# gabegrand/VQA-Counterexamples

Hardware: AMD Instinct MI355X
Metric: VQA-CX triplets/sec (24 candidates each), NeuralCX training step (higher is better)
Workload: dtype f32; 1 GPU; configs[1]: NeuralCX MLP train step (fwd+listwise loss/recall+bwd+Adam), synthetic 2048-d feats, 24 candidates, batch 512 per GPU (weak scaling: global batch 512), H=256, L=1, dropout 0.25, fp32; global_batch=512, per_rank_batch=512, candidates=24, dim_h=256, n_layers=1, parallelism=dp1, feature_table_rows=82783

## Files before the change

### include/neuralcx.h

```cpp
#ifndef NEURALCX_H
#define NEURALCX_H

#include <stddef.h>
#include <stdint.h>

#ifdef __cplusplus
extern "C" {
#endif

#define NCX_OK            0
#define NCX_E_NULL       -1
#define NCX_E_DIMS       -2
#define NCX_E_WORKSPACE  -3
#define NCX_E_FLAGS      -4
#define NCX_E_UNSUPPORTED -5
#define NCX_E_COMM       -6

#define NCX_F_V_MULT   (1u << 0)
#define NCX_F_V_DIST   (1u << 1)
#define NCX_F_V_RANK   (1u << 2)
#define NCX_F_A_EMB    (1u << 3)
#define NCX_F_ALL      (NCX_F_V_MULT | NCX_F_V_DIST | NCX_F_V_RANK | NCX_F_A_EMB)
#define NCX_F_BF16     (1u << 4)
#define NCX_F_REUSE_GT (1u << 5)
// ... 102 lines not shown
    int32_t act_v, act_q;
} ncx_mutan_params;

size_t ncx_vqa_workspace_bytes(const ncx_dims* d, const ncx_mutan_params* m);

int ncx_vqa_forward(const ncx_dims* d, const float* feats, const int32_t* img_idx, const float* q_emb,
                    const ncx_mutan_params* m, void* workspace, size_t workspace_bytes,
                    float* z_orig, float* z_knns, float* a_knns, float* a_orig, void* stream);

size_t ncx_knn_workspace_bytes(int32_t n, int32_t block_rows);
int ncx_knn(const float* table, int32_t n, const float* queries, int32_t nq, int32_t dv, int32_t k,
            int32_t norms_ready, void* workspace, size_t workspace_bytes, int64_t* out_idx, float* out_dist,
            void* stream);

size_t ncx_cosine_gram_workspace_bytes(int32_t A, int32_t da);
int ncx_cosine_gram(const float* emb, int32_t A, int32_t da, void* ws, size_t ws_bytes, float* gram, void* stream);
int ncx_semantic_scores(const float* a_knns, const int32_t* aid, int32_t B, int32_t K, int32_t A, const float* gram,
                        float lam, float* scores, float* raw, int32_t* bad_id_flag, void* stream);

#define NCX_GEMM_GT 0
#define NCX_GEMM_SH 1
#define NCX_GEMM_MAIN 2
#define NCX_GEMM_FWD_L 3
#define NCX_GEMM_DW1C 4
#define NCX_GEMM_DW1S 5
#define NCX_GEMM_DE 6
#define NCX_GEMM_DW1AK 7
#define NCX_GEMM_DAGT 8
#define NCX_GEMM_DWL 9
#define NCX_GEMM_DXL 10
int ncx_profile_begin(uint32_t gemm_mask , int32_t max_launches);
int ncx_profile_end(float* ms, int32_t* ids, int32_t cap);
int ncx_profile_stamps(unsigned long long* stamps, int64_t words);
int ncx_plan_query(const ncx_dims* d, int32_t gemm_id, int32_t* out6);
int ncx_wgmap_check(int32_t tiles_m, int32_t tiles_n, int32_t S);

const char* ncx_version(void);

#ifdef __cplusplus
}
#endif
#endif
```

### vqa-counterexamples_amd/csrc/ncx_api.hip

```cpp
#include "ncx_internal.h"
#include "ncx_dwred.h"
#include "ncx_bf16.h"
#include <stdlib.h>
#include <stdio.h>
#include <atomic>

namespace ncx {

template <int CTRL> __device__ __forceinline__ float dpp_mov(float v) {
    return __builtin_bit_cast(float, __builtin_amdgcn_update_dpp(0, __builtin_bit_cast(int, v), CTRL, 0xF, 0xF, false));
}
__device__ __forceinline__ float lane_bcast(float v, int lane) {
    return __builtin_bit_cast(float, __builtin_amdgcn_readlane(__builtin_bit_cast(int, v), lane));
}
__device__ __forceinline__ float wave_sum(float v) {
    v += dpp_mov<0xB1>(v); v += dpp_mov<0x4E>(v); v += dpp_mov<0x141>(v); v += dpp_mov<0x140>(v);
    return (lane_bcast(v, 0) + lane_bcast(v, 16)) + (lane_bcast(v, 32) + lane_bcast(v, 48));
}
__device__ __forceinline__ float wave_max(float v) {
    v = fmaxf(v, dpp_mov<0xB1>(v)); v = fmaxf(v, dpp_mov<0x4E>(v)); v = fmaxf(v, dpp_mov<0x141>(v)); v = fmaxf(v, dpp_mov<0x140>(v));
    return fmaxf(fmaxf(lane_bcast(v, 0), lane_bcast(v, 16)), fmaxf(lane_bcast(v, 32), lane_bcast(v, 48)));
}

__device__ __forceinline__ u16 f32_to_bf16(float x) { return __builtin_bit_cast(u16, (__bf16)x); }
// ... 717 lines not shown
    if (const char* e = hook_env("NCX_SMALL_COLS")) narrow = atoll(e);
    if (S <= 1 || cols > narrow) return S;
    int mult = 2;
    if (const char* e = hook_env("NCX_SMALL_MULT")) mult = atoi(e) > 0 ? atoi(e) : 1;
    long long sp = (long long)S * mult;
    const long long smax = ksteps / 8 > 1 ? ksteps / 8 : 1;
    if (sp > smax) sp = smax;
    return (int)(sp < S ? S : sp);
}

static void list_uses(const ncx_dims& d, GemmUse* u) {
    const long long M = (long long)d.B * d.K, H = d.H;
    const bool aemb = d.flags & NCX_F_A_EMB;
    const long long cand_k = ks(d.dv) * ((d.flags & NCX_F_V_MULT) ? 2 : 1) + ks(d.K + 1) + ks(d.dz) + (aemb ? ks(d.A) : ks(d.da));
    const long long cand_cols = (long long)d.dv * ((d.flags & NCX_F_V_MULT) ? 2 : 1) + d.K + 1 + d.dz + (aemb ? d.A : d.da);
    const long long sh_k = ks(d.dv) + ks(d.dq) + ks(d.dz) + ks(d.da);
    const long long sh_cols = (long long)d.dv + d.dq + d.dz + d.da;
    u[U_GT]    = {FORM_NT, H, d.A, ks(d.da), false};
    u[U_SH]    = {FORM_NT, d.B, H, sh_k, false};
    u[U_MAIN]  = {FORM_NT, M, H, cand_k, true};
    u[U_FWD_L] = {FORM_NT, M, H, ks(H), true};
    u[U_DW1C]  = {FORM_TN, H, cand_cols, ks(M), false};
    u[U_DW1S]  = {FORM_TN, H, sh_cols, ks(d.B), false};
    u[U_DE]    = {FORM_TN, d.A, d.da, 2 * ks(H), false};
    u[U_DW1AK] = {FORM_NN, H, d.da, ks(d.A), false};
    u[U_DAGT]  = {FORM_NN, 1, 1, 1, false};
    u[U_DWL]   = {FORM_TN, H, H, ks(M), false};
    u[U_DXL]   = {FORM_NN, M, H, ks(H), false};
    const bool hooks = experiment_hooks_on();
    for (int i = 0; i < U_COUNT; ++i) {
        const bool km = dw_km_supported(d) && !(d.flags & NCX_F_BF16);
        const bool tn8 = dw_tn8_supported(d);
        const long long segs_c[5] = {km ? 0 : d.dv, (!km && (d.flags & NCX_F_V_MULT)) ? d.dv : 0, tn8 ? 0 : d.K + 1, tn8 ? 0 : d.dz, tn8 ? 0 : (aemb ? d.A : d.da)};
        const bool tn8s = tn8 || dw_tn8_shapes_ok(d);
        const long long segs_s[5] = {tn8s ? 0 : d.dv, tn8s ? 0 : d.dq, tn8s ? 0 : d.dz, tn8s ? 0 : d.da, 0};
        const bool grouped = i == U_DW1C || i == U_DW1S;
        auto grouped_tiles = [&](int bm, int bn) {
            const long long* sg = i == U_DW1C ? segs_c : segs_s;
            long long t = 0;
            for (int q = 0; q < 5; ++q) t += cdiv(H, bm) * cdiv(sg[q], bn);
            return t;
        };
        if (grouped && grouped_tiles(64, 64) == 0) {
            u[i].plan.cfg = CFG_128x64; u[i].plan.split = 1;
        } else if (grouped) {
            u[i].plan = plan_from_tiles(FORM_TN, grouped_tiles(128, 128), grouped_tiles(64, 64), u[i].ksteps, false);
            if (i == U_DW1C && H >= 128 && u[i].plan.split > 1) {
                u[i].plan.cfg = CFG_128x64;
                const long long slots = (long long)occupancy_tn(CFG_128x64) * num_cus();
                long long sp = cdiv(3 * slots, grouped_tiles(128, 64));
                const long long smax = u[i].ksteps / 24 > 1 ? u[i].ksteps / 24 : 1;
                if (sp > 8) sp = 8;
                u[i].plan.split = (int)(sp > smax ? smax : sp < 1 ? 1 : sp);
            }
        } else {
            u[i].plan = plan_gemm(u[i].form, u[i].M, u[i].N, u[i].ksteps, u[i].allow96);
        }
        if (i == U_MAIN || i == U_FWD_L || i == U_DXL) u[i].plan.split = 1;
        if (hooks) {
            char name[32];
            snprintf(name, sizeof name, "NCX_CFG_%d", i);
            const char* c = getenv(name);
            if (c) u[i].plan.cfg = atoi(c);
            snprintf(name, sizeof name, "NCX_SPLIT_%d", i);
            const char* e = getenv(name);
            if (e && i != U_MAIN && i != U_FWD_L && i != U_DXL) u[i].plan.split = atoi(e) > 1 ? atoi(e) : 1;
        }
        int bm, bn; cfg_tile(u[i].plan.cfg, bm, bn);
        long long tiles = cdiv(u[i].M, bm) * cdiv(u[i].N, bn);
        if (grouped) tiles = grouped_tiles(bm, bn);
        u[i].tiles = tiles;
        const int S = u[i].plan.split > 1 ? u[i].plan.split : 1;
        long long wgs = 0;
        if (grouped) {
            const long long* sg = i == U_DW1C ? segs_c : segs_s;
            for (int q = 0; q < 5; ++q)
                if (sg[q] > 0) wgs += WgMap{(int)cdiv(H, bm), (int)cdiv(sg[q], bn), i == U_DW1C ? dw1c_seg_split(sg[q], S, u[i].ksteps) : S}.count();
        } else {
            wgs = WgMap{(int)cdiv(u[i].M, bm), (int)cdiv(u[i].N, bn), S}.count();
        }
        u[i].wgs = wgs;
        u[i].slab_elems = S > 1 ? wgs * bm * bn : 0;
    }
    u[U_DW1S].plan.cfg = u[U_DW1C].plan.cfg;
    {
        int bm, bn; cfg_tile(u[U_DW1C].plan.cfg, bm, bn);
        const bool tn8 = dw_tn8_shapes_ok(d);
        const long long segs_s[4] = {tn8 ? 0 : d.dv, tn8 ? 0 : d.dq, tn8 ? 0 : d.dz, tn8 ? 0 : d.da};
        const int S = u[U_DW1S].plan.split > 1 ? u[U_DW1S].plan.split : 1;
        u[U_DW1S].tiles = 0; u[U_DW1S].wgs = 0;
        for (int q = 0; q < 4; ++q) {
            if (segs_s[q] == 0) continue;
            u[U_DW1S].tiles += cdiv(H, bm) * cdiv(segs_s[q], bn);
            u[U_DW1S].wgs += WgMap{(int)cdiv(H, bm), (int)cdiv(segs_s[q], bn), S}.count();
        }
        u[U_DW1C].slab_elems = (u[U_DW1C].wgs + u[U_DW1S].wgs) * bm * bn;
        u[U_DW1S].slab_elems = 0;
    }
}

WsLayout ws_layout(const ncx_dims& d) {
    WsLayout w{};
    const size_t M = (size_t)d.B * d.K, H = d.H;
    size_t off = 0;
    auto take = [&](size_t bytes) { size_t o = off; off = align_up(off + bytes, 256); return o; };
    w.idx_k = take(M * 4); w.idx_o = take(M * 4); w.idx_ob = take((size_t)d.B * 4);
    w.mx = take(M * 4); w.inv = take(M * 4);
    w.ldm = pad_to(d.K + 1, 4);
    w.ldgt = (d.flags & NCX_F_BF16) ? d.A : pad_to(d.A, 32);
    w.misc = take(M * w.ldm * 4);
    w.gt = take(H * w.ldgt * 4);
    w.sh = take((size_t)d.B * H * 4);
    for (int l = 0; l < 3; ++l) w.h[l] = l < d.L ? take(M * H * 4) : 0;
    w.dpre[0] = take(M * H * 4);
    w.dpre[1] = d.L >= 2 ? take(M * H * 4) : 0;
    w.dsh = take((size_t)d.B * H * 4);
    w.dgt = take(2 * H * d.A * 4);
    w.dagt = w.dgt + H * d.A * 4;
    w.dgtT = take((size_t)2 * d.A * pad_to(d.H, 4) * 4);
    w.w1aT = take((size_t)2 * d.da * pad_to(d.H, 32) * 4);
// ... 628 lines not shown
            prob(in->q_emb, d.dq, 0, d.dq, g->w1 + o.q_emb);
            prob(in->z_orig, d.dz, 0, d.dz, g->w1 + o.z_orig);
            if (aemb) prob(p->answer_embedding, d.da, 2, d.da, g->w1 + o.a_gt);
            else      prob(in->a_emb_gt, d.da, 0, d.da, g->w1 + o.a_gt);
            rc = dw_tn8(d, tp, np, 0, false, true, idx_ob, aemb ? in->answer_aids : nullptr, slab, w.slab_bytes, s); if (rc) return rc;
        } else
        if (want_rest && !tn8) {
            add_s(x_gather(in->feats, d.dv, idx_ob, d.B, d.dv), g->w1 + o.v_orig);
            add_s(x_plain(in->q_emb, d.dq, d.B, d.dq), g->w1 + o.q_emb);
            add_s(x_plain(in->z_orig, d.dz, d.B, d.dz), g->w1 + o.z_orig);
            add_s(aemb ? x_gather(p->answer_embedding, d.da, in->answer_aids, d.B, d.da) : x_plain(in->a_emb_gt, d.da, d.B, d.da),
                  g->w1 + o.a_gt);
        }
        a.nseg = n;
        FixupArgs fix_tn{};
        if (km_merge) a.defer_fix = &fix_tn;
        if (n > 0) { rc = run_gemm(U_DW1C, a, FORM_TN, u[U_DW1C].plan, slab, w.slab_bytes, nullptr, s); if (rc) return rc; }
        if (km_merge && !km_reduced) {
            rc = prof_open(U_DW1C, s); if (rc) return rc;
            rc = dw_km_finish(d, (const float*)(ws + w.km_slab), g->w1 + o.v_other, g->w1 + o.v_mult, din, &fix_tn, u[U_DW1C].plan.cfg, s);
            if (rc) return rc;
            rc = prof_close(U_DW1C, s); if (rc) return rc;
        }
        if (!(d.flags & NCX_F_V_MULT) && do2) {
            hipLaunchKernelGGL(k_zero_cols, dim3((unsigned)cdiv((long long)H * d.dv, 256)), dim3(256), 0, s, g->w1 + o.v_mult, H, din, d.dv);
            NCX_HIP_TRY(hipGetLastError());
        }
    }
    if (aemb) {
        SideStream* ss = km_deferred ? side_stream() : nullptr;
        hipStream_t se = ss ? ss->s : s;
        FixupArgs fix_ak{};
        Tn8ReduceArgs red_ak{};
        const bool tn8_ak = dw_tn8_supported(d) && emb_nt && !ss;
        if (ss) { rc = side_fork(ss, s); if (rc) return rc; }
        const bool bf16e = d.flags & NCX_F_BF16;
        const Bf16Emb bm = bf16e ? bf16_emb_layout(d, ws + w.bf_emb) : Bf16Emb{};
        if (do2 && bf16e) {
            rc = prof_open(U_DW1AK, se); if (rc) return rc;
            rc = bf16_dw1ak(d, bm, dgt, g->w1, se); if (rc) return rc;
            rc = prof_close(U_DW1AK, se); if (rc) return rc;
        } else if (do2 && tn8_ak) {
            Tn8Prob q{};
            q.A = (const float*)(ws + w.dgtT2); q.rows = pad_to(d.A, 32); q.rows_valid = d.A; q.X = p->answer_embedding; q.ldx = d.da; q.N = d.da;
            q.out = g->w1 + o.a_other; q.ldo = din; q.n_valid = d.da;
            rc = prof_open(U_DW1AK, se); if (rc) return rc;
            rc = dw_tn8_products(d, &q, 1, 0, false, true, nullptr, nullptr, slab, w.slab_bytes, &red_ak, se); if (rc) return rc;
            if (!(do1 && emb_nt)) { rc = dw_reduce_km_tn8(nullptr, true, &red_ak, se); if (rc) return rc; red_ak.n_tiles_total = 0; }
            rc = prof_close(U_DW1AK, se); if (rc) return rc;
        } else if (do2) {
            GemmArgs a{}; a.mode = MODE_CHAIN; a.nseg = 1; a.M = H;
            a.a[0] = x_plain(dgt, d.A, H, d.A); a.b[0] = x_plain(p->answer_embedding, d.da, d.A, d.da); a.klen[0] = d.A;
            a.out[0] = g->w1 + o.a_other; a.ldo[0] = din; a.n_cols[0] = d.da;
            if (do1 && emb_nt && u[U_DW1AK].plan.cfg == CFG_64x64 && !hook_env("NCX_NO_MERGE_FIX")) a.defer_fix = &fix_ak;
            rc = run_gemm(U_DW1AK, a, FORM_NN, u[U_DW1AK].plan, ss ? (float*)(ws + w.slab2) : slab,
                          ss ? w.slab2_bytes : w.slab_bytes, nullptr, se); if (rc) return rc;
        }
        if (do1 && emb_nt) {
            EmbPrepArgs ea{};
            ea.dsh = dsh; ea.aid = in->answer_aids; ea.dggtT = dagtT; ea.B = d.B; ea.H = H; ea.A = d.A; ea.Hp4 = Hp4;
            const float* srcs[3] = {dgt, p->w1 + o.a_other, p->w1 + o.a_gt};
            float* dsts[3] = {dgtT, w1akT, w1agtT};
            const long long ldss[3] = {d.A, din, din};
            const int colss[3] = {tn8_ak ? 0 : d.A, d.da, d.da}, ldds[3] = {Hp4, Hp32, Hp32};
            int tiles = 0;
            for (int e = 0; e < 3; ++e) {
                ea.src[e] = srcs[e]; ea.dst[e] = dsts[e]; ea.lds_[e] = ldss[e]; ea.cols[e] = colss[e]; ea.ldd[e] = ldds[e]; ea.dcols[e] = ldds[e];
// ... 234 lines not shown
    int dev = 0;
    NCX_HIP_TRY(hipGetDevice(&dev));
    if (dev < 0 || dev >= 16) return NCX_E_DIMS;
    if (!stamps) { g_stamps[dev].ptr.store(nullptr, std::memory_order_release); g_stamps[dev].words.store(0, std::memory_order_release); }
    else { g_stamps[dev].ptr.store(nullptr, std::memory_order_release); g_stamps[dev].words.store(words, std::memory_order_release);
           g_stamps[dev].ptr.store(stamps, std::memory_order_release); }
    return NCX_OK;
}

int ncx_wgmap_check(int32_t tiles_m, int32_t tiles_n, int32_t S) {
    if (tiles_m < 1 || tiles_n < 1 || S < 1 || (long long)tiles_m * tiles_n * S > (1 << 24)) return NCX_E_DIMS;
    const WgMap w{tiles_m, tiles_n, S};
    const int total = tiles_m * tiles_n * S, count = w.count();
    if (count < total) return 1;
    unsigned char* seen = (unsigned char*)calloc((size_t)total, 1);
    if (!seen) return NCX_E_NULL;
    int bad = 0, nvalid = 0;
    for (int lw = 0; lw < count && !bad; ++lw) {
        int tm = -1, tn = -1, z = -1;
        if (!w.decode(lw, tm, tn, z)) continue;
        ++nvalid;
        if (tm < 0 || tm >= tiles_m || tn < 0 || tn >= tiles_n || z < 0 || z >= S) { bad = 2; break; }
        if (w.encode(tm, tn, z) != lw) { bad = 3; break; }
        unsigned char& f = seen[((size_t)z * tiles_m + tm) * tiles_n + tn];
        if (f) { bad = 4; break; }
        f = 1;
    }
    if (!bad && nvalid != total) bad = 5;
    free(seen);
    return bad;
}

int ncx_plan_query(const ncx_dims* d, int32_t gemm_id, int32_t* out6) {
    if (check_dims(d) != NCX_OK || !out6 || gemm_id < 0 || gemm_id >= U_COUNT) return NCX_E_DIMS;
    GemmUse u[U_COUNT];
    list_uses(*d, u);
    out6[0] = u[gemm_id].form; out6[1] = (int32_t)u[gemm_id].M; out6[2] = (int32_t)u[gemm_id].N;
    out6[3] = (int32_t)u[gemm_id].ksteps; out6[4] = u[gemm_id].plan.cfg; out6[5] = u[gemm_id].plan.split;
    const bool fast = (gemm_id == U_MAIN && main_fwd_dims_ok(*d)) || (gemm_id == U_FWD_L && hidden_fwd_dims_ok(*d) && !(d->flags & NCX_F_BF16));
    if (fast) {
        const long long M = (long long)d->B * d->K, T = u[gemm_id].ksteps;
        const int sp = main_split(M, d->H, T);
        const bool vfold = gemm_id == U_MAIN && (d->flags & NCX_F_V_MULT) && (d->K == 24 || (d->K == 48 && main_fold_rows(M, d->H) >= 96)) && d->dv % 32 == 0 && d->dv >= 64 && sp == 1;
        const long long tiles96 = ((M + 95) / 96) * ((d->H + 127) / 128);
        out6[4] = vfold ? (main_fold_rows(M, d->H) == 192 ? 8 : (main_fold_rows(M, d->H) == 96 || d->K == 48) ? 7 : 6) : (sp == 1 && tiles96 * 10 >= (long long)num_cus() * 9) ? CFG_96x128 : 5;
        out6[5] = sp;
    }
    return NCX_OK;
}

}
```

### vqa-counterexamples_amd/csrc/ncx_dwred.h

```cpp
#pragma once
#include "ncx_internal.h"

namespace ncx {

constexpr int TN8_BM = 256, TN8_BN = 64, TN8_BK = 32, TN8_T = 512;

struct KmReduceArgs { const float* slab; int nz, H, dv; long long din; float* g_vother; float* g_vmult; int nblk; };
template <bool VEC>
__device__ __forceinline__ void km_reduce_body(const KmReduceArgs& r, int blk) {
    constexpr int W = VEC ? 4 : 1;
    typedef float vec __attribute__((ext_vector_type(VEC ? 4 : 1)));
    const long long i = ((long long)blk * 256 + threadIdx.x) * W, n = (long long)r.H * r.dv;
    if (i >= n) return;
    const int h = (int)(i / r.dv), c = (int)(i - (long long)h * r.dv);
    vec vk[DW_KM_SPLIT], vm[DW_KM_SPLIT];
#pragma unroll
    for (int z = 0; z < DW_KM_SPLIT; ++z) {
        const int zz = z < r.nz ? z : r.nz - 1;
        vk[z] = *(const vec*)(r.slab + ((long long)zz * 2 + 0) * n + i);
        vm[z] = *(const vec*)(r.slab + ((long long)zz * 2 + 1) * n + i);
    }
    vec sk = vk[0], sm = vm[0];
#pragma unroll
    for (int z = 1; z < DW_KM_SPLIT; ++z) { const vec zero = {}; sk += z < r.nz ? vk[z] : zero; sm += z < r.nz ? vm[z] : zero; }
#pragma unroll
    for (int j = 0; j < W; ++j) {
        r.g_vother[(long long)h * r.din + c + j] = sk[j];
        r.g_vmult[(long long)h * r.din + c + j] = sm[j];
    }
}

struct Tn8ReduceArgs {
    Tn8Prob p[TN8_MAX_PROB];
    int np, n_al, tiles_m, S, al_wgs, R, do_al, do_rest;
    int rest_tiles[TN8_MAX_PROB], rest_steps[TN8_MAX_PROB], rest_tile0[TN8_MAX_PROB], rest_pre[TN8_MAX_PROB + 1];
    int al_tiles, n_tiles_total;
    const float* slab;
};
__device__ __forceinline__ void tn8_reduce_body(const Tn8ReduceArgs& r, int blk) {
    int tile_blk = blk >> 3;
    const int rgp = blk & 7;
    int prob, tile, s_first, s_count, s_stride = 1;
    if (r.do_al && tile_blk < r.al_tiles) {
        prob = 0; tile = tile_blk; s_first = tile * r.S; s_count = r.S;
    } else {
        if (r.do_al) tile_blk -= r.al_tiles;
        prob = r.n_al;
        while (prob + 1 < r.np && tile_blk >= r.rest_tile0[prob + 1]) ++prob;
        tile = tile_blk - r.rest_tile0[prob];
        const long long g0 = (long long)r.rest_pre[prob] + (long long)tile * r.rest_steps[prob], g1 = g0 + r.rest_steps[prob];
        const int w0 = (int)(g0 / r.R), w1 = (int)((g1 - 1) / r.R);
        s_first = r.al_wgs + r.rest_tile0[prob] + tile + w0; s_count = w1 - w0 + 1;
    }
    const Tn8Prob& p = r.p[prob];
    const int tm = tile % r.tiles_m, tn = tile / r.tiles_m;
    __shared__ float tn8_tt[32][TN8_BN + 1];
#pragma unroll
    for (int it = 0; it < 2; ++it) {
        const int f = threadIdx.x + 256 * it, row = rgp * 32 + (f >> 4), c = 4 * (f & 15);
        const float* src = r.slab + (long long)s_first * (TN8_BM * TN8_BN) + row * TN8_BN + c;
        f32x4 sum = {0.f, 0.f, 0.f, 0.f};
        for (int z = 0; z < s_count; z += 8) {
            f32x4 v[8];
#pragma unroll
            for (int j = 0; j < 8; ++j) v[j] = *(const f32x4*)(src + (long long)min(z + j, s_count - 1) * s_stride * (TN8_BM * TN8_BN));
#pragma unroll
            for (int j = 0; j < 8; ++j) sum += z + j < s_count ? v[j] : f32x4{0.f, 0.f, 0.f, 0.f};
        }
        const int h = tm * TN8_BM + row, n = tn * TN8_BN + c;
        float* o = p.out + (long long)h * p.ldo + n;
#pragma unroll
        for (int j = 0; j < 4; ++j) if (n + j < p.n_valid) o[j] = sum[j];
        if (p.outT) {
#pragma unroll
            for (int j = 0; j < 4; ++j) tn8_tt[f >> 4][c + j] = sum[j];
        }
    }
    if (p.outT) {
        __syncthreads();
        const int nl = threadIdx.x >> 2, hq = (threadIdx.x & 3) * 8;
        const int n = tn * TN8_BN + nl, h0 = tm * TN8_BM + rgp * 32 + hq;
        if (n < p.n_valid + p.padT2) {
            float v[8];
#pragma unroll
            for (int j = 0; j < 8; ++j) v[j] = n < p.n_valid ? tn8_tt[hq + j][nl] : 0.f;
#pragma unroll
            for (int j = 0; j < 8; ++j) {
                if (n < p.n_valid) p.outT[(long long)n * p.ldT + h0 + j] = v[j];
                if (p.outT2) p.outT2[(long long)n * p.ldT + h0 + j] = v[j];
            }
        }
    }
}

int dw_tn8_products(const ncx_dims& d, const Tn8Prob* probs, int np, int n_al, bool do_al, bool do_rest, const int* idx_ob, const int* aid,
                    float* slab, size_t slab_bytes, Tn8ReduceArgs* red, hipStream_t s);
int dw_reduce_km_tn8(const KmReduceArgs* km, bool km_vec, const Tn8ReduceArgs* tn, hipStream_t s);
KmReduceArgs dw_km_reduce_args(const ncx_dims& d, const float* slab, float* g_vother, float* g_vmult, long long din, bool* vec);

}
```

### vqa-counterexamples_amd/csrc/ncx_dwtn.hip

```cpp
#include <hip/hip_runtime.h>
#include <stdint.h>
#include <stdlib.h>
#include <type_traits>
#include "ncx_internal.h"
#include "ncx_dwred.h"

namespace ncx {

constexpr int TN8_PA = 256, TN8_PB = 80;
constexpr int TN8_MAX_SEG = 16;
constexpr int TN8_SEG_WORDS = 16;

typedef const __attribute__((address_space(1))) float* tn_gfptr;
typedef const __attribute__((address_space(1))) f32x4u* tn_gf4ptr;

struct Tn8Args {
    Tn8Prob p[TN8_MAX_PROB];
    int np, n_al;
    int H, tiles_m, B;
    int S, al_wgs, al_tiles_n;
    int R;
    int do_al, do_rest;
    int rest_tiles[TN8_MAX_PROB], rest_steps[TN8_MAX_PROB], rest_tile0[TN8_MAX_PROB];
    int rest_pre[TN8_MAX_PROB + 1];
    const int* idx_ob; const int* aid;
    float* slab;
    int n_slots;
};

struct Tn8Seg {
    unsigned long long a_ptr;
    unsigned long long x_ptr;
    unsigned long long l_ptr;
    int ldx;
    int soft;
    int gsel;
    int n0, ncl;
    int t0;
    int vbeg, vend;
    int slot;
    int rv;
};
static_assert(sizeof(Tn8Seg) == TN8_SEG_WORDS * 4, "segment record");

// ... 478 lines not shown
#pragma unroll
            for (int p = 0; p < 3; ++p) afB[p] = zero8;
            flush();
            ++qc;
            if (qc < nseg) { vend_c = segs[qc].vend; slot_c = segs[qc].slot; }
        }
    };
    typedef std::integral_constant<int, 0> M0; typedef std::integral_constant<int, 1> M1; typedef std::integral_constant<int, 2> M2;
    auto pair = [&](auto mode_c, int v) __attribute__((always_inline)) {
        if (v + 3 >= l_vend) loader_switch(v + 3);
        step(S0{}, mode_c, v);
        if (v + 4 >= l_vend) loader_switch(v + 4);
        step(S1{}, mode_c, v + 1);
    };
    int v = 0;
    if constexpr (SPLIT) {
        const int nal = (a.do_al && w < a.al_wgs && segs[0].slot == w) ? segs[0].vend : 0;
        const int nA = nal > 1 ? (nal - 1) & ~1 : 0, nB = nal & ~1;
        for (; v + 1 < V && v < nA; v += 2) pair(M1{}, v);
        for (; v + 1 < V && v < nB; v += 2) pair(M0{}, v);
        for (; v + 1 < V; v += 2) pair(M2{}, v);
        if (v < V) { if (v + 3 >= l_vend) loader_switch(v + 3); step(S0{}, M0{}, v); }
    } else {
        for (; v + 1 < V; v += 2) pair(M0{}, v);
        if (v < V) { if (v + 3 >= l_vend) loader_switch(v + 3); step(S0{}, M0{}, v); }
    }
}


static inline int tn8_cdiv(long long a, long long b) { return (int)((a + b - 1) / b); }

constexpr int TN6_MAX_B = 2048;
bool dw_tn8_x6(const ncx_dims& d) { return (d.flags & NCX_F_X6) && d.B <= TN6_MAX_B && !hook_env("NCX_NO_X6"); }
bool dw_tn8_supported(const ncx_dims& d) { return !(d.flags & NCX_F_BF16) && dw_tn8_shapes_ok(d); }
bool dw_tn8_shapes_ok(const ncx_dims& d) {
    if (hook_env("NCX_NO_TN8")) return false;
    const long long M = (long long)d.B * d.K;
    if (d.H % TN8_BM != 0 || d.B % TN8_BK != 0 || M % TN8_BK != 0 || d.B > 4096 || d.B < 128) return false;
    if (d.dv % 4 || d.dq % 4 || d.dz % 4 || d.da % 4 || d.A % 4) return false;
    const long long lim = (1ll << 32) - 65536;
    if ((long long)d.n_img * d.dv * 4 >= lim || M * (long long)(d.A > d.da ? d.A : d.da) * 4 >= lim || M * (long long)d.H * 4 >= lim || (long long)d.A * d.da * 4 >= lim) return false;
    return true;
}

struct Tn8Plan { int grid, S, al_wgs, al_tiles, R, n_slots, rest_tiles_total; };
static Tn8Plan tn8_plan(const ncx_dims& d, const Tn8Prob* p, int np, int n_al, int* rest_tiles, int* rest_steps, int* rest_tile0, int* rest_pre) {
    Tn8Plan pl{};
    const int cus = num_cus(), tiles_m = d.H / TN8_BM;
    pl.grid = cus;
    if (n_al) {
        pl.al_tiles = tiles_m * tn8_cdiv(p[0].N, TN8_BN);
        const int steps = p[0].rows / TN8_BK;
        int S = cus / pl.al_tiles; if (S < 1) S = 1;
        while (S > 1 && steps / S < 8) --S;
        pl.S = S; pl.al_wgs = pl.al_tiles * S;
        if (pl.al_wgs > pl.grid) pl.grid = pl.al_wgs;
    } else { pl.S = 1; pl.al_wgs = 0; pl.al_tiles = 0; }
    long long g = 0; int t0 = 0;
    for (int i = 0; i < TN8_MAX_PROB; ++i) { rest_tiles[i] = 0; rest_steps[i] = 1; rest_tile0[i] = 0; rest_pre[i] = 0; }
    for (int i = n_al; i < np; ++i) {
        rest_tiles[i] = tiles_m * tn8_cdiv(p[i].N, TN8_BN); rest_steps[i] = p[i].rows / TN8_BK; rest_tile0[i] = t0; rest_pre[i] = (int)g;
        t0 += rest_tiles[i]; g += (long long)rest_tiles[i] * rest_steps[i];
    }
    for (int i = np; i <= TN8_MAX_PROB; ++i) rest_pre[i] = (int)g;
    for (int i = 0; i < n_al; ++i) rest_pre[i] = 0;
    pl.rest_tiles_total = t0;
    pl.R = g > 0 ? tn8_cdiv(g, pl.grid) : 1;
    pl.n_slots = pl.al_wgs + t0 + pl.grid;
    return pl;
}

size_t dw_tn8_slab_bytes(const ncx_dims& d) {
    if (!dw_tn8_shapes_ok(d)) return 0;
    const int cus = num_cus(), tiles_m = d.H / TN8_BM;
    const bool aemb = d.flags & NCX_F_A_EMB, bf16 = d.flags & NCX_F_BF16;
    long long al_wgs = 0;
    if (aemb && !bf16) { const int t = tiles_m * tn8_cdiv(d.A, TN8_BN); int S = cus / t; if (S < 1) S = 1; al_wgs = (long long)t * S; }
    long long rest_tiles = 0;
    const int cols[7] = {(aemb || bf16) ? 0 : d.da, bf16 ? 0 : d.dz, bf16 ? 0 : pad_to(d.K + 1, 4), d.dv, d.dq, d.dz, d.da};
    for (int i = 0; i < 7; ++i) if (cols[i]) rest_tiles += (long long)tiles_m * tn8_cdiv(cols[i], TN8_BN);
    const long long grid = al_wgs > cus ? al_wgs : cus;
    return (size_t)(al_wgs + rest_tiles + grid) * TN8_BM * TN8_BN * 4;
}

static int tn8_fill(const ncx_dims& d, const Tn8Prob* probs, int np, int n_al, bool do_al, bool do_rest, Tn8Args& a, Tn8ReduceArgs& r,
                    float* slab, size_t slab_bytes, Tn8Plan& pl) {
    if (np < 1 || np > TN8_MAX_PROB || n_al < 0 || n_al > 1 || n_al > np) return NCX_E_DIMS;
    for (int i = 0; i < np; ++i) {
        if (probs[i].rows % TN8_BK || probs[i].N < 4 || probs[i].N % 4 || probs[i].ldx % 4) return NCX_E_DIMS;
        if (probs[i].gsel && probs[i].rows != d.B) return NCX_E_DIMS;
        a.p[i] = probs[i]; r.p[i] = probs[i];
    }
    pl = tn8_plan(d, probs, np, n_al, a.rest_tiles, a.rest_steps, a.rest_tile0, a.rest_pre);
    if ((size_t)pl.n_slots * TN8_BM * TN8_BN * 4 > slab_bytes) return NCX_E_WORKSPACE;
    int min_steps = 1 << 30;
    for (int i = n_al; i < np; ++i) min_steps = a.rest_steps[i] < min_steps ? a.rest_steps[i] : min_steps;
    if (np > n_al && 1 + pl.R / min_steps + 2 > TN8_MAX_SEG) return NCX_E_DIMS;
    a.np = np; a.n_al = n_al; a.H = d.H; a.tiles_m = d.H / TN8_BM; a.B = d.B;
    a.S = pl.S; a.al_wgs = pl.al_wgs; a.al_tiles_n = n_al ? tn8_cdiv(probs[0].N, TN8_BN) : 0; a.R = pl.R;
    a.do_al = do_al && n_al; a.do_rest = do_rest && np > n_al;
    a.slab = slab; a.n_slots = pl.n_slots;
    r.np = np; r.n_al = n_al; r.tiles_m = a.tiles_m; r.S = pl.S; r.al_wgs = pl.al_wgs; r.R = pl.R; r.do_al = a.do_al; r.do_rest = a.do_rest;
    for (int i = 0; i < TN8_MAX_PROB; ++i) { r.rest_tiles[i] = a.rest_tiles[i]; r.rest_steps[i] = a.rest_steps[i]; r.rest_tile0[i] = a.rest_tile0[i]; }
    for (int i = 0; i <= TN8_MAX_PROB; ++i) r.rest_pre[i] = a.rest_pre[i];
    r.al_tiles = pl.al_tiles; r.slab = slab;
    r.n_tiles_total = (a.do_al ? pl.al_tiles : 0) + (a.do_rest ? pl.rest_tiles_total : 0);
    return NCX_OK;
}

int dw_tn8_products(const ncx_dims& d, const Tn8Prob* probs, int np, int n_al, bool do_al, bool do_rest, const int* idx_ob, const int* aid,
                    float* slab, size_t slab_bytes, Tn8ReduceArgs* red, hipStream_t s) {
    Tn8Args a{}; Tn8ReduceArgs r{}; Tn8Plan pl;
    int rc = tn8_fill(d, probs, np, n_al, do_al, do_rest, a, r, slab, slab_bytes, pl);
    if (rc) return rc;
    *red = r;
    if (!a.do_al && !a.do_rest) { red->n_tiles_total = 0; return NCX_OK; }
    a.idx_ob = idx_ob; a.aid = aid;
    if (dw_tn8_x6(d)) {
        const int lds = 2 * TN6_BUF + TN8_MAX_SEG * (int)sizeof(Tn8Seg) + 2 * (d.B + 32) * 4;
        static DevMask attr6{0};
        bool split6 = !hook_env("NCX_TN8_NO_SPLIT");
        for (int i = 0; i < np; ++i) split6 = split6 && ((probs[i].lse != nullptr) == (i < n_al));
        static DevMask attr6s{0};
        if (split6) {
            NCX_HIP_TRY(set_max_lds_once(attr6s, (const void*)k_dw_tn8_x6<true>, 2 * TN6_BUF + TN8_MAX_SEG * (int)sizeof(Tn8Seg) + 2 * (TN6_MAX_B + 32) * 4));
            hipLaunchKernelGGL(k_dw_tn8_x6<true>, dim3(pl.grid), dim3(TN8_T), lds, s, a);
        } else {
            NCX_HIP_TRY(set_max_lds_once(attr6, (const void*)k_dw_tn8_x6<false>, 2 * TN6_BUF + TN8_MAX_SEG * (int)sizeof(Tn8Seg) + 2 * (TN6_MAX_B + 32) * 4));
            hipLaunchKernelGGL(k_dw_tn8_x6<false>, dim3(pl.grid), dim3(TN8_T), lds, s, a);
        }
// ... 47 lines not shown
```

### vqa-counterexamples_amd/csrc/ncx_internal.h

```cpp
#pragma once
#include "ncx_common.h"
#include "ncx_gemm.h"

namespace ncx {

enum TileCfg : int { CFG_64x64 = 0, CFG_128x128 = 1, CFG_96x128 = 2, CFG_96x64 = 3, CFG_128x64 = 4 };
enum GemmForm : int { FORM_NT = 0, FORM_TN = 1, FORM_NN = 2 };

int run_gemm_nt(GemmArgs& a, int cfg, hipStream_t s);
int run_fixup2(const FixupArgs& a, const FixupArgs& b, int cfg, hipStream_t s);
int run_gemm_nt_fold(GemmArgs& a, hipStream_t s);
int run_gemm_tn(GemmArgs& a, int cfg, hipStream_t s);
int run_gemm_nn(GemmArgs& a, int cfg, hipStream_t s);
int occupancy_nt(int cfg);
int occupancy_tn(int cfg);
int occupancy_nn(int cfg);

struct SegOffsets {
    int v_orig, v_other, v_mult, v_dist, v_rank, q_emb, z_orig, z_other, a_gt, a_other, din;
};
static inline SegOffsets seg_offsets(const ncx_dims& d) {
    SegOffsets o; int c = 0;
    o.v_orig = c;  c += d.dv;
    o.v_other = c; c += d.dv;
// ... 57 lines not shown
    int kind, klen;
};
struct MainArgs {
    MainSeg seg[MAIN_MAX_SEG]; int nseg, M, N, split; float* out; long long ldo; EpiArgs epi;
    float* slab;
    float* dist_out; long long ld_dist;
    unsigned long long* stamps;
    int x6;
};
int main_forward(MainArgs& a, hipStream_t s);
int main_split(long long M, long long N, long long T);
int main_fold_rows_eff(long long M, long long N, int rowdiv);
int main_fold_rows(long long M, long long N);

constexpr int DW_KM_SPLIT = 8;
bool dw_km_supported(const ncx_dims& d);
size_t dw_km_slab_bytes(const ncx_dims& d);
int dw_km(const ncx_dims& d, const float* dpre, const float* feats, const int* idx_k, const int* idx_o, float* slab,
          float* g_vother, float* g_vmult, long long din, hipStream_t s, bool finish = true);
int dw_km_finish(const ncx_dims& d, const float* slab, float* g_vother, float* g_vmult, long long din, const FixupArgs* fix, int fix_cfg,
                 hipStream_t s);
constexpr int TN8_MAX_PROB = 8;
struct Tn8Prob {
    const float* A;
    const float* X; long long ldx;
    const float* lse;
    int gsel;
    int rows, N;
    float* out; long long ldo; int n_valid;
    int rows_valid;
    float* outT; float* outT2; long long ldT; int padT2;
};
bool dw_tn8_supported(const ncx_dims& d);
bool dw_tn8_shapes_ok(const ncx_dims& d);
size_t dw_tn8_slab_bytes(const ncx_dims& d);
int dw_tn8(const ncx_dims& d, const Tn8Prob* probs, int np, int n_al, bool do_al, bool do_rest, const int* idx_ob, const int* aid,
           float* slab, size_t slab_bytes, hipStream_t s);
bool mutan_fold_supported(const ncx_dims& d, const ncx_mutan_params& m);
int mutan_fold(const ncx_dims& d, const ncx_mutan_params& m, const float* xv, const float* hq, float* z_orig, float* z_knns, hipStream_t s);
WsLayout ws_layout(const ncx_dims& d);
__host__ __device__ static inline int pad_to(int x, int m) { return (x + m - 1) / m * m; }
static inline bool main_fwd_extents_ok(const ncx_dims& d) {
    const long long lim = (1ll << 32) - 65536, M = (long long)d.B * d.K, wa = d.A > d.da ? d.A : d.da;
    return (long long)d.n_img * d.dv * 4 < lim && M * wa * 4 < lim && M * (long long)d.H * 4 < lim && M * (long long)d.dz * 4 < lim && (long long)d.A * wa * 4 < lim &&
           (long long)d.H * (2ll * d.dv + d.dq + 2ll * d.dz + 2ll * d.da + d.K + 2) * 4 < lim;
}
static inline bool main_fwd_dims_ok(const ncx_dims& d) {
    return d.dv % 4 == 0 && d.dz % 4 == 0 && ((d.flags & NCX_F_A_EMB) ? d.A : d.da) % 4 == 0 && !(d.flags & NCX_F_BF16) && main_fwd_extents_ok(d);
}
static inline bool hidden_fwd_dims_ok(const ncx_dims& d) { return d.H % 4 == 0 && main_fwd_extents_ok(d); }
constexpr uint32_t NCX_F_PRIV_DIST_IN_MAIN = 1u << 30;


}
```

Measured before the change: 650,900 triplets/s.

## Tighten TN8 eligibility checks and vectorize the split-K reduce with swizzled LDS transpose

The TN8 split-K reduction now loads both row groups per thread together, unrolled four deep over splits instead of eight. The transpose goes through a flat, XOR-swizzled shared buffer, and transposed outputs are written with 16-byte vector stores when alignment allows. Eligibility for TN8 now also checks that the segment count fits under TN8_MAX_SEG, so kernel launch no longer fails late with a dims error. A plan-query hook is added for inspection. The planner's use of TN8 for shared-weight paths is changed to match the new supported predicates, which may alter tiling plans.

```diff
diff --git a/include/neuralcx.h b/include/neuralcx.h
--- a/include/neuralcx.h
+++ b/include/neuralcx.h
@@ -158,6 +158,7 @@
 int ncx_profile_begin(uint32_t gemm_mask , int32_t max_launches);
 int ncx_profile_end(float* ms, int32_t* ids, int32_t cap);
 int ncx_profile_stamps(unsigned long long* stamps, int64_t words);
+#define NCX_PLAN_TN8 100
 int ncx_plan_query(const ncx_dims* d, int32_t gemm_id, int32_t* out6);
 int ncx_wgmap_check(int32_t tiles_m, int32_t tiles_n, int32_t S);
 
diff --git a/vqa-counterexamples_amd/csrc/ncx_api.hip b/vqa-counterexamples_amd/csrc/ncx_api.hip
--- a/vqa-counterexamples_amd/csrc/ncx_api.hip
+++ b/vqa-counterexamples_amd/csrc/ncx_api.hip
@@ -773,7 +773,7 @@
         const bool km = dw_km_supported(d) && !(d.flags & NCX_F_BF16);
         const bool tn8 = dw_tn8_supported(d);
         const long long segs_c[5] = {km ? 0 : d.dv, (!km && (d.flags & NCX_F_V_MULT)) ? d.dv : 0, tn8 ? 0 : d.K + 1, tn8 ? 0 : d.dz, tn8 ? 0 : (aemb ? d.A : d.da)};
-        const bool tn8s = tn8 || dw_tn8_shapes_ok(d);
+        const bool tn8s = tn8 || ((d.flags & NCX_F_BF16) && dw_tn8_shapes_ok(d));
         const long long segs_s[5] = {tn8s ? 0 : d.dv, tn8s ? 0 : d.dq, tn8s ? 0 : d.dz, tn8s ? 0 : d.da, 0};
         const bool grouped = i == U_DW1C || i == U_DW1S;
         auto grouped_tiles = [&](int bm, int bn) {
@@ -826,7 +826,7 @@
     u[U_DW1S].plan.cfg = u[U_DW1C].plan.cfg;
     {
         int bm, bn; cfg_tile(u[U_DW1C].plan.cfg, bm, bn);
-        const bool tn8 = dw_tn8_shapes_ok(d);
+        const bool tn8 = dw_tn8_supported(d) || ((d.flags & NCX_F_BF16) && dw_tn8_shapes_ok(d));
         const long long segs_s[4] = {tn8 ? 0 : d.dv, tn8 ? 0 : d.dq, tn8 ? 0 : d.dz, tn8 ? 0 : d.da};
         const int S = u[U_DW1S].plan.split > 1 ? u[U_DW1S].plan.split : 1;
         u[U_DW1S].tiles = 0; u[U_DW1S].wgs = 0;
@@ -1521,7 +1521,7 @@
         hipStream_t se = ss ? ss->s : s;
         FixupArgs fix_ak{};
         Tn8ReduceArgs red_ak{};
-        const bool tn8_ak = dw_tn8_supported(d) && emb_nt && !ss;
+        const bool tn8_ak = dw_tn8_ak_supported(d) && emb_nt && !ss;
         if (ss) { rc = side_fork(ss, s); if (rc) return rc; }
         const bool bf16e = d.flags & NCX_F_BF16;
         const Bf16Emb bm = bf16e ? bf16_emb_layout(d, ws + w.bf_emb) : Bf16Emb{};
@@ -1822,6 +1822,7 @@
 }
 
 int ncx_plan_query(const ncx_dims* d, int32_t gemm_id, int32_t* out6) {
+    if (check_dims(d) == NCX_OK && out6 && gemm_id == NCX_PLAN_TN8) { dw_tn8_plan_info(*d, out6); return NCX_OK; }
     if (check_dims(d) != NCX_OK || !out6 || gemm_id < 0 || gemm_id >= U_COUNT) return NCX_E_DIMS;
     GemmUse u[U_COUNT];
     list_uses(*d, u);
diff --git a/vqa-counterexamples_amd/csrc/ncx_dwred.h b/vqa-counterexamples_amd/csrc/ncx_dwred.h
--- a/vqa-counterexamples_amd/csrc/ncx_dwred.h
+++ b/vqa-counterexamples_amd/csrc/ncx_dwred.h
@@ -54,40 +54,50 @@
     }
     const Tn8Prob& p = r.p[prob];
     const int tm = tile % r.tiles_m, tn = tile / r.tiles_m;
-    __shared__ float tn8_tt[32][TN8_BN + 1];
+    __shared__ __attribute__((aligned(16))) float tn8_tt[32 * TN8_BN];
+    const int f = threadIdx.x, c = 4 * (f & 15);
+    const float* src = r.slab + (long long)s_first * (TN8_BM * TN8_BN) + (rgp * 32 + (f >> 4)) * TN8_BN + c;
+    f32x4 sum[2] = {{0.f, 0.f, 0.f, 0.f}, {0.f, 0.f, 0.f, 0.f}};
+    for (int z = 0; z < s_count; z += 4) {
+        f32x4 v[2][4];
+#pragma unroll
+        for (int it = 0; it < 2; ++it)
+#pragma unroll
+            for (int j = 0; j < 4; ++j) v[it][j] = *(const f32x4*)(src + it * 16 * TN8_BN + (long long)min(z + j, s_count - 1) * s_stride * (TN8_BM * TN8_BN));
+#pragma unroll
+        for (int it = 0; it < 2; ++it)
+#pragma unroll
+            for (int j = 0; j < 4; ++j) sum[it] += z + j < s_count ? v[it][j] : f32x4{0.f, 0.f, 0.f, 0.f};
+    }
 #pragma unroll
     for (int it = 0; it < 2; ++it) {
-        const int f = threadIdx.x + 256 * it, row = rgp * 32 + (f >> 4), c = 4 * (f & 15);
-        const float* src = r.slab + (long long)s_first * (TN8_BM * TN8_BN) + row * TN8_BN + c;
-        f32x4 sum = {0.f, 0.f, 0.f, 0.f};
-        for (int z = 0; z < s_count; z += 8) {
-            f32x4 v[8];
-#pragma unroll
-            for (int j = 0; j < 8; ++j) v[j] = *(const f32x4*)(src + (long long)min(z + j, s_count - 1) * s_stride * (TN8_BM * TN8_BN));
-#pragma unroll
-            for (int j = 0; j < 8; ++j) sum += z + j < s_count ? v[j] : f32x4{0.f, 0.f, 0.f, 0.f};
-        }
-        const int h = tm * TN8_BM + row, n = tn * TN8_BN + c;
+        const int rl = (f >> 4) + 16 * it, h = tm * TN8_BM + rgp * 32 + rl, n = tn * TN8_BN + c;
         float* o = p.out + (long long)h * p.ldo + n;
 #pragma unroll
-        for (int j = 0; j < 4; ++j) if (n + j < p.n_valid) o[j] = sum[j];
-        if (p.outT) {
-#pragma unroll
-            for (int j = 0; j < 4; ++j) tn8_tt[f >> 4][c + j] = sum[j];
-        }
+        for (int j = 0; j < 4; ++j) if (n + j < p.n_valid) o[j] = sum[it][j];
+        if (p.outT) *(f32x4*)(tn8_tt + rl * TN8_BN + (((f & 15) ^ ((rl >> 3) << 1)) << 2)) = sum[it];
     }
     if (p.outT) {
         __syncthreads();
         const int nl = threadIdx.x >> 2, hq = (threadIdx.x & 3) * 8;
         const int n = tn * TN8_BN + nl, h0 = tm * TN8_BM + rgp * 32 + hq;
         if (n < p.n_valid + p.padT2) {
-            float v[8];
+            f32x4 v[2];
 #pragma unroll
-            for (int j = 0; j < 8; ++j) v[j] = n < p.n_valid ? tn8_tt[hq + j][nl] : 0.f;
+            for (int j = 0; j < 8; ++j)
+                v[j >> 2][j & 3] = n < p.n_valid ? tn8_tt[(hq + j) * TN8_BN + ((((nl >> 2) ^ ((hq >> 3) << 1)) << 2) | (nl & 3))] : 0.f;
+            const bool vec = (p.ldT & 3) == 0 && (((uintptr_t)p.outT | (uintptr_t)p.outT2) & 15) == 0;
+            float* oT = p.outT + (long long)n * p.ldT + h0;
+            float* oT2 = p.outT2 ? p.outT2 + (long long)n * p.ldT + h0 : nullptr;
+            if (vec) {
+                if (n < p.n_valid) { *(f32x4*)oT = v[0]; *(f32x4*)(oT + 4) = v[1]; }
+                if (oT2) { *(f32x4*)oT2 = v[0]; *(f32x4*)(oT2 + 4) = v[1]; }
+            } else {
 #pragma unroll
-            for (int j = 0; j < 8; ++j) {
-                if (n < p.n_valid) p.outT[(long long)n * p.ldT + h0 + j] = v[j];
-                if (p.outT2) p.outT2[(long long)n * p.ldT + h0 + j] = v[j];
+                for (int j = 0; j < 8; ++j) {
+                    if (n < p.n_valid) oT[j] = v[j >> 2][j & 3];
+                    if (oT2) oT2[j] = v[j >> 2][j & 3];
+                }
             }
         }
     }
diff --git a/vqa-counterexamples_amd/csrc/ncx_dwtn.hip b/vqa-counterexamples_amd/csrc/ncx_dwtn.hip
--- a/vqa-counterexamples_amd/csrc/ncx_dwtn.hip
+++ b/vqa-counterexamples_amd/csrc/ncx_dwtn.hip
@@ -1,6 +1,7 @@
 #include <hip/hip_runtime.h>
 #include <stdint.h>
 #include <stdlib.h>
+#include <string.h>
 #include <type_traits>
 #include "ncx_internal.h"
 #include "ncx_dwred.h"
@@ -10,6 +11,7 @@
 constexpr int TN8_PA = 256, TN8_PB = 80;
 constexpr int TN8_MAX_SEG = 16;
 constexpr int TN8_SEG_WORDS = 16;
+enum { TN8_LIST_MAIN = 0, TN8_LIST_AK = 1, TN8_LIST_SHARED = 2 };
 
 typedef const __attribute__((address_space(1))) float* tn_gfptr;
 typedef const __attribute__((address_space(1))) f32x4u* tn_gf4ptr;
@@ -554,8 +556,14 @@
 
 constexpr int TN6_MAX_B = 2048;
 bool dw_tn8_x6(const ncx_dims& d) { return (d.flags & NCX_F_X6) && d.B <= TN6_MAX_B && !hook_env("NCX_NO_X6"); }
-bool dw_tn8_supported(const ncx_dims& d) { return !(d.flags & NCX_F_BF16) && dw_tn8_shapes_ok(d); }
-bool dw_tn8_shapes_ok(const ncx_dims& d) {
+static int tn8_list_pieces(const ncx_dims& d, int which);
+static bool dw_tn8_dims_ok(const ncx_dims& d);
+bool dw_tn8_supported(const ncx_dims& d) { return !(d.flags & NCX_F_BF16) && dw_tn8_shapes_ok(d) && tn8_list_pieces(d, TN8_LIST_MAIN) <= TN8_MAX_SEG; }
+bool dw_tn8_ak_supported(const ncx_dims& d) {
+    return dw_tn8_supported(d) && (d.flags & NCX_F_A_EMB) && tn8_list_pieces(d, TN8_LIST_AK) <= TN8_MAX_SEG;
+}
+bool dw_tn8_shapes_ok(const ncx_dims& d) { return dw_tn8_dims_ok(d) && tn8_list_pieces(d, TN8_LIST_SHARED) <= TN8_MAX_SEG; }
+static bool dw_tn8_dims_ok(const ncx_dims& d) {
     if (hook_env("NCX_NO_TN8")) return false;
     const long long M = (long long)d.B * d.K;
     if (d.H % TN8_BM != 0 || d.B % TN8_BK != 0 || M % TN8_BK != 0 || d.B > 4096 || d.B < 128) return false;
@@ -592,6 +600,58 @@
     return pl;
 }
 
+static int tn8_max_pieces(const Tn8Plan& pl, const int* rest_steps, int np, int n_al) {
+    if (np <= n_al) return n_al;
+    int min_steps = 1 << 30;
+    for (int i = n_al; i < np; ++i) min_steps = rest_steps[i] < min_steps ? rest_steps[i] : min_steps;
+    return 1 + pl.R / min_steps + 2;
+}
+
+static int tn8_list(const ncx_dims& d, int which, Tn8Prob* tp, int* n_al) {
+    const int M = d.B * d.K;
+    int np = 0;
+    auto prob = [&](int rows, int N) { tp[np] = Tn8Prob{}; tp[np].rows = rows; tp[np].N = N; ++np; };
+    *n_al = 0;
+    if (which == TN8_LIST_AK) { prob(pad_to(d.A, 32), d.da); return np; }
+    if (which == TN8_LIST_MAIN) {
+        if (d.flags & NCX_F_A_EMB) { prob(M, d.A); *n_al = 1; }
+        else prob(M, d.da);
+        prob(M, d.dz);
+        prob(M, pad_to(d.K + 1, 4));
+    }
+    prob(d.B, d.dv); prob(d.B, d.dq); prob(d.B, d.dz); prob(d.B, d.da);
+    return np;
+}
+static int tn8_list_pieces_uncached(const ncx_dims& d, int which);
+static int tn8_list_pieces(const ncx_dims& d, int which) {
+    if (!dw_tn8_dims_ok(d)) return TN8_MAX_SEG + 1;
+    static thread_local struct { ncx_dims d; int r; bool valid; } memo[3];
+    if (memo[which].valid && !memcmp(&memo[which].d, &d, sizeof d)) return memo[which].r;
+    const int r = tn8_list_pieces_uncached(d, which);
+    memo[which].d = d; memo[which].r = r; memo[which].valid = true;
+    return r;
+}
+static int tn8_list_pieces_uncached(const ncx_dims& d, int which) {
+    Tn8Prob tp[TN8_MAX_PROB]; int n_al;
+    const int np = tn8_list(d, which, tp, &n_al);
+    int rt[TN8_MAX_PROB], rs[TN8_MAX_PROB], r0[TN8_MAX_PROB], rp[TN8_MAX_PROB + 1];
+    const Tn8Plan pl = tn8_plan(d, tp, np, n_al, rt, rs, r0, rp);
+    return tn8_max_pieces(pl, rs, np, n_al);
+}
+void dw_tn8_plan_info(const ncx_dims& d, int32_t* out6) {
+    out6[0] = dw_tn8_supported(d) ? 1 : 0; out6[1] = tn8_list_pieces(d, TN8_LIST_MAIN);
+    out6[2] = dw_tn8_ak_supported(d) ? 1 : 0; out6[3] = (d.flags & NCX_F_A_EMB) ? tn8_list_pieces(d, TN8_LIST_AK) : 0;
+    out6[4] = TN8_MAX_SEG;
+    int grid = 0;
+    if (dw_tn8_dims_ok(d)) {
+        Tn8Prob tp[TN8_MAX_PROB]; int n_al;
+        const int np = tn8_list(d, TN8_LIST_MAIN, tp, &n_al);
+        int rt[TN8_MAX_PROB], rs[TN8_MAX_PROB], r0[TN8_MAX_PROB], rp[TN8_MAX_PROB + 1];
+        grid = tn8_plan(d, tp, np, n_al, rt, rs, r0, rp).grid;
+    }
+    out6[5] = grid;
+}
+
 size_t dw_tn8_slab_bytes(const ncx_dims& d) {
     if (!dw_tn8_shapes_ok(d)) return 0;
     const int cus = num_cus(), tiles_m = d.H / TN8_BM;
@@ -615,9 +675,7 @@
     }
     pl = tn8_plan(d, probs, np, n_al, a.rest_tiles, a.rest_steps, a.rest_tile0, a.rest_pre);
     if ((size_t)pl.n_slots * TN8_BM * TN8_BN * 4 > slab_bytes) return NCX_E_WORKSPACE;
-    int min_steps = 1 << 30;
-    for (int i = n_al; i < np; ++i) min_steps = a.rest_steps[i] < min_steps ? a.rest_steps[i] : min_steps;
-    if (np > n_al && 1 + pl.R / min_steps + 2 > TN8_MAX_SEG) return NCX_E_DIMS;
+    if (tn8_max_pieces(pl, a.rest_steps, np, n_al) > TN8_MAX_SEG) return NCX_E_DIMS;
     a.np = np; a.n_al = n_al; a.H = d.H; a.tiles_m = d.H / TN8_BM; a.B = d.B;
     a.S = pl.S; a.al_wgs = pl.al_wgs; a.al_tiles_n = n_al ? tn8_cdiv(probs[0].N, TN8_BN) : 0; a.R = pl.R;
     a.do_al = do_al && n_al; a.do_rest = do_rest && np > n_al;
diff --git a/vqa-counterexamples_amd/csrc/ncx_internal.h b/vqa-counterexamples_amd/csrc/ncx_internal.h
--- a/vqa-counterexamples_amd/csrc/ncx_internal.h
+++ b/vqa-counterexamples_amd/csrc/ncx_internal.h
@@ -113,6 +113,8 @@
     float* outT; float* outT2; long long ldT; int padT2;
 };
 bool dw_tn8_supported(const ncx_dims& d);
+bool dw_tn8_ak_supported(const ncx_dims& d);
+void dw_tn8_plan_info(const ncx_dims& d, int32_t* out6);
 bool dw_tn8_shapes_ok(const ncx_dims& d);
 size_t dw_tn8_slab_bytes(const ncx_dims& d);
 int dw_tn8(const ncx_dims& d, const Tn8Prob* probs, int np, int n_al, bool do_al, bool do_rest, const int* idx_ob, const int* aid,
```

Result: no change. 653,600 triplets/s, median of 6 (+0.4%).
